# cvigilv/SimSpread.jl

Measured on AMD Instinct MI355X. Metric: predicted edges/sec + achieved HBM GB/s, W*R SpMM, higher is better.
Workload: dtype f32

## Files before the change

simspread.jl_amd/csrc/assemble.hip:

```cpp
#include <cstdlib>
#include <cstring>
#include <hip/hip_runtime.h>
#include <rocprim/rocprim.hpp>

#include "graph.hpp"

namespace ss {

static inline int grid_for(int64_t work, int block, int cap = 256 * 16) {
  int64_t g = ceil_div(work, block);
  if (g < 1) g = 1;
  if (g > cap) g = cap;
  return (int)g;
}

__global__ void scan_tail_kernel(const int* in, int* out, int64_t n) { out[n] = out[n - 1] + in[n - 1]; }

static int exclusive_scan_int(const int* in, int* out, int64_t n) {
  hipStream_t st = ctx().stream;
  if (n == 0) {
    SS_HIP(hipMemsetAsync(out, 0, sizeof(int), st));
    return SS_OK;
  }
  size_t bytes = 0;
// ... 289 lines not shown
  for (int64_t i = (int64_t)blockIdx.x * blockDim.x + threadIdx.x; i < n; i += (int64_t)gridDim.x * blockDim.x)
    atomicAdd(&hist[keys[i]], 1);
}

template <class T>
__global__ void gather_transpose_kernel(const int* __restrict__ perm, const int* __restrict__ rowid,
                                        const T* __restrict__ val, int64_t n, int* __restrict__ oidx,
                                        T* __restrict__ oval) {
  for (int64_t i = (int64_t)blockIdx.x * blockDim.x + threadIdx.x; i < n; i += (int64_t)gridDim.x * blockDim.x) {
    const int p = perm[i];
    oidx[i] = rowid[p];
    oval[i] = val[p];
  }
}

template <class T>
int csr_transpose(const DevCsr<T>& in, DevCsr<T>& out) {
  hipStream_t st = ctx().stream;
  out.rows = in.cols;
  out.cols = in.rows;
  out.nnz = in.nnz;
  out.binary = in.binary;
  SS_TRY(out.ptr.alloc(out.rows + 1));
  SS_TRY(out.idx.alloc(in.nnz));
  SS_TRY(out.val.alloc(in.nnz));
  const int64_t n = in.nnz;
  DevBuf<int> hist;
  SS_TRY(hist.alloc(out.rows + 1));
  SS_HIP(hipMemsetAsync(hist.p, 0, (out.rows + 1) * sizeof(int), st));
  if (n == 0) {
    SS_HIP(hipMemsetAsync(out.ptr.p, 0, (out.rows + 1) * sizeof(int), st));
    return SS_OK;
  }
  DevBuf<int> rowid, iota, keys_out, perm;
  SS_TRY(rowid.alloc(n));
  SS_TRY(iota.alloc(n));
  SS_TRY(keys_out.alloc(n));
  SS_TRY(perm.alloc(n));
  hipLaunchKernelGGL(expand_rows_kernel, dim3(grid_for(in.rows * 64, 256)), dim3(256), 0, st, in.ptr.p, in.rows,
                     rowid.p, iota.p);
  SS_LAUNCH_CHECK();
  int bits = 1;
  while ((1LL << bits) < in.cols && bits < 32) ++bits;
  size_t bytes = 0;
  SS_HIP(rocprim::radix_sort_pairs(nullptr, bytes, in.idx.p, keys_out.p, iota.p, perm.p, (size_t)n, 0u,
                                   (unsigned)bits, st));
  DevBuf<unsigned char> tmp;
  SS_TRY(tmp.alloc(bytes));
  SS_HIP(rocprim::radix_sort_pairs(tmp.p, bytes, in.idx.p, keys_out.p, iota.p, perm.p, (size_t)n, 0u,
                                   (unsigned)bits, st));
  hipLaunchKernelGGL(histogram_kernel, dim3(grid_for(n, 256)), dim3(256), 0, st, in.idx.p, n, hist.p);
  SS_LAUNCH_CHECK();
  SS_TRY(exclusive_scan_int(hist.p, out.ptr.p, out.rows));
  hipLaunchKernelGGL(gather_transpose_kernel<T>, dim3(grid_for(n, 256)), dim3(256), 0, st, perm.p, rowid.p,
                     in.val.p, n, out.idx.p, out.val.p);
  SS_LAUNCH_CHECK();
  SS_HIP(hipStreamSynchronize(st));
  return SS_OK;
}

__global__ void sell_width_kernel(const int* __restrict__ ptr, const int* __restrict__ idx, int64_t rows, int KC,
                                  int nslices, int nchunks, const int* __restrict__ vs, const int* __restrict__ ve,
                                  int* __restrict__ widthq) {
  const int lane = threadIdx.x & 63;
  const int64_t wave = ((int64_t)blockIdx.x * blockDim.x + threadIdx.x) >> 6;
  if (wave >= (int64_t)nslices * nchunks) return;
  const int c = (int)(wave / nslices), s = (int)(wave % nslices);
  const int64_t pos = (int64_t)s * 64 + lane;
  int n = 0;
  if (pos < rows) {
    int lo = vs ? vs[pos] : ptr[pos], hi = ve ? ve[pos] : ptr[pos + 1];
    const int64_t k0 = (int64_t)c * KC, k1 = k0 + KC;
    int a = lo, b = hi;
    while (a < b) { const int m = (a + b) >> 1; if (idx[m] < k0) a = m + 1; else b = m; }
    const int first = a;
    b = hi;
    while (a < b) { const int m = (a + b) >> 1; if (idx[m] < k1) a = m + 1; else b = m; }
    n = a - first;
  }
  for (int o = 32; o > 0; o >>= 1) { const int t = __shfl_xor(n, o); n = t > n ? t : n; }
  if (lane == 0) widthq[wave] = (n + 3) >> 2;
}

template <class T>
__global__ void sell_fill_kernel(const int* __restrict__ ptr, const int* __restrict__ idx, const T* __restrict__ val,
                                 int64_t rows, int KC, int nslices, int nchunks, const int* __restrict__ off,
                                 const int* __restrict__ vs, const int* __restrict__ ve,
                                 unsigned short* __restrict__ sidx, T* __restrict__ sval) {
  const int lane = threadIdx.x & 63;
  const int64_t wave = ((int64_t)blockIdx.x * blockDim.x + threadIdx.x) >> 6;
  if (wave >= (int64_t)nslices * nchunks) return;
  const int c = (int)(wave / nslices), s = (int)(wave % nslices);
  const int64_t pos = (int64_t)s * 64 + lane;
  int first = 0, n = 0;
  const int64_t k0 = (int64_t)c * KC, k1 = k0 + KC;
  if (pos < rows) {
    int lo = vs ? vs[pos] : ptr[pos], hi = ve ? ve[pos] : ptr[pos + 1];
    int a = lo, b = hi;
    while (a < b) { const int m = (a + b) >> 1; if (idx[m] < k0) a = m + 1; else b = m; }
    first = a;
    b = hi;
    while (a < b) { const int m = (a + b) >> 1; if (idx[m] < k1) a = m + 1; else b = m; }
    n = a - first;
  }
  const int o = off[wave], oe = off[wave + 1];
  for (int u = o; u < oe; ++u) {
    const int64_t base = ((int64_t)u * 64 + lane) * 4;
#pragma unroll
    for (int e = 0; e < 4; ++e) {
      const int p = (u - o) * 4 + e;
      const bool in = p < n;
      sidx[base + e] = in ? (unsigned short)(idx[first + p] - k0) : (unsigned short)KC;
      if (sval) sval[base + e] = in ? val[first + p] : T(0);
    }
  }
}

__device__ __forceinline__ void b128_group_of_lane(int lane, int& grp, int& gi) {
  const int l = lane & 31;
  int g, i;
  if (l < 4) { g = 0; i = l; }
  else if (l < 12) { g = 1; i = l - 4; }
  else if (l < 16) { g = 0; i = l - 8; }
  else if (l < 20) { g = 1; i = l - 8; }
  else if (l < 28) { g = 0; i = l - 12; }
  else { g = 1; i = l - 16; }
  grp = g + ((lane >> 5) << 1);
  gi = i;
}
__device__ __forceinline__ int b128_lane_of_group(int grp, int gi) {
  const int g = grp & 1;
  int l;
  if (g == 0) l = gi < 4 ? gi : (gi < 8 ? gi + 8 : gi + 12);
  else l = gi < 8 ? gi + 4 : (gi < 12 ? gi + 8 : gi + 16);
  return l + ((grp >> 1) << 5);
}

template <class T>
__global__ void __launch_bounds__(64) sell_fill_sched_kernel(const int* __restrict__ ptr, const int* __restrict__ idx,
                                                             const T* __restrict__ val, int64_t rows, int KC,
                                                             int nslices, int nchunks, const int* __restrict__ off,
                                                             const int* __restrict__ vs, const int* __restrict__ ve,
                                                             int* __restrict__ perm, unsigned short* __restrict__ sidx,
                                                             T* __restrict__ sval, int ncls, int npid) {
  __shared__ unsigned short cnt[64][17];
  __shared__ int cur[64][17];
  const int lane = threadIdx.x;
  const int64_t wave = blockIdx.x;
  const int c = (int)(wave / nslices), s = (int)(wave % nslices);
  const int64_t pos = (int64_t)s * 64 + lane;
  int first = 0, n = 0;
  const int64_t k0 = (int64_t)c * KC, k1 = k0 + KC;
  if (pos < rows) {
    int lo = vs ? vs[pos] : ptr[pos], hi = ve ? ve[pos] : ptr[pos + 1];
    int a = lo, b = hi;
    while (a < b) { const int m = (a + b) >> 1; if (idx[m] < k0) a = m + 1; else b = m; }
    first = a;
    b = hi;
    while (a < b) { const int m = (a + b) >> 1; if (idx[m] < k1) a = m + 1; else b = m; }
    n = a - first;
  }
  for (int q = 0; q < ncls; ++q) cnt[lane][q] = 0;
  for (int x = 0; x < n; ++x) cnt[lane][(idx[first + x] - k0) & (ncls - 1)]++;
  int run = first;
  for (int q = 0; q < ncls; ++q) { cur[lane][q] = run; run += cnt[lane][q]; }
  for (int x = 0; x < n; ++x) {
    const int q = (int)((idx[first + x] - k0) & (ncls - 1));
    perm[cur[lane][q]++] = first + x;
  }
  for (int q = 0; q < ncls; ++q) cur[lane][q] -= cnt[lane][q];

  int grp, gi;
  b128_group_of_lane(lane, grp, gi);
  const int o = off[wave], oe = off[wave + 1];
  int left = n;
  unsigned have = 0;
  for (int q = 0; q < ncls; ++q) have |= (cnt[lane][q] > 0 ? 1u : 0u) << q;
  const int psh = (lane & (npid - 1)) * ncls;
  for (int p = 0; p < (oe - o) * 4; ++p) {
    unsigned claimed = 0;
    int mine = -1;
    bool done = left == 0;
    for (int it = 0; it < 16; ++it) {
      if (__ballot(!done) == 0ull) break;
      const int rest = left > 4095 ? 4095 : left;
      int key = done ? 0x7fffffff : ((__popc(have & ~(claimed >> psh)) << 20) | ((4095 - rest) << 4) | gi);
#pragma unroll
      for (int m2 = 1; m2 < 16; m2 <<= 1) {
        const int other = __shfl(key, b128_lane_of_group(grp, gi ^ m2));
        key = other < key ? other : key;
      }
      const bool any = key != 0x7fffffff;
      const int wgi = key & 15;
      int choice = -1;
      if (any && !done && gi == wgi) {
        int best = -1, bestc = 0;
        for (int q = 0; q < ncls; ++q) {
          const int cq = cnt[lane][q];
          if (cq > bestc && !((claimed >> (psh + q)) & 1u)) { best = q; bestc = cq; }
        }
        if (best < 0)
          for (int q = 0; q < ncls; ++q) {
            const int cq = cnt[lane][q];
            if (cq > bestc) { best = q; bestc = cq; }
          }
        choice = best;
        mine = best;
        done = true;
      }
      const int wl = b128_lane_of_group(grp, wgi);
      const int ch = __shfl(choice, wl);
      if (any && ch >= 0) claimed |= 1u << ((wl & (npid - 1)) * ncls + ch);
    }
    const int64_t base = ((int64_t)(o + (p >> 2)) * 64 + lane) * 4 + (p & 3);
    if (mine >= 0) {
      const int e = perm[cur[lane][mine]];
      cur[lane][mine]++;
      cnt[lane][mine]--;
      if (cnt[lane][mine] == 0) have &= ~(1u << mine);
      --left;
      sidx[base] = (unsigned short)(idx[e] - k0);
      if (sval) sval[base] = val[e];
    } else {
      int q = 0;
      while (q < ncls - 1 && ((claimed >> (psh + q)) & 1u)) ++q;
      sidx[base] = (unsigned short)(KC + ((q - KC) & (ncls - 1)));
      if (sval) sval[base] = T(0);
    }
  }
}

__global__ void vrow_parts_kernel(const int* __restrict__ ptr, int64_t rows, int lmax, int* __restrict__ nparts) {
  for (int64_t i = (int64_t)blockIdx.x * blockDim.x + threadIdx.x; i < rows; i += (int64_t)gridDim.x * blockDim.x) {
    const int len = ptr[i + 1] - ptr[i];
    nparts[i] = len > lmax ? (len + lmax - 1) / lmax : 1;
  }
}
__global__ void vrow_fill_kernel(const int* __restrict__ ptr, const int* __restrict__ vfirst, int64_t rows, int lmax,
                                 int* __restrict__ vstart, int* __restrict__ vlen, int* __restrict__ iota) {
  for (int64_t r = (int64_t)blockIdx.x * blockDim.x + threadIdx.x; r < rows; r += (int64_t)gridDim.x * blockDim.x) {
    const int lo = ptr[r], hi = ptr[r + 1];
    for (int v = vfirst[r], p = 0; v < vfirst[r + 1]; ++v, ++p) {
      const int b = lo + p * lmax;
      const int e = (b + lmax < hi) ? b + lmax : hi;
      vstart[v] = b;
      vlen[v] = e > b ? e - b : 0;
      iota[v] = v;
    }
  }
}
__global__ void vrow_place_kernel(const int* __restrict__ perm, const int* __restrict__ vstart,
                                  const int* __restrict__ vlen, int64_t n, int* __restrict__ vs, int* __restrict__ ve,
                                  int* __restrict__ inv) {
  for (int64_t i = (int64_t)blockIdx.x * blockDim.x + threadIdx.x; i < n; i += (int64_t)gridDim.x * blockDim.x) {
    const int v = perm[i];
    vs[i] = vstart[v];
    ve[i] = vstart[v] + vlen[v];
    inv[v] = (int)i;
  }
}

template <class T>
int sell_build(const DevCsr<T>& in, int KCmax, DevSell<T>& out, int qt) {
  hipStream_t st = ctx().stream;
  if (qt <= 0) qt = sell_tile_width<T>();
  const int rowb = qt * (int)sizeof(T);
  if (rowb != 16 && rowb != 32) return fail(SS_EINVAL, "SELL tile rows must be 16 or 32 bytes");
  out.qt = qt;
  const int ncls = 256 / rowb, npid = rowb / 16;
  if (KCmax < 1 || KCmax > 65520) return fail(SS_EINVAL, "SELL chunk size out of range");
  out.rows = in.rows;
  out.cols = in.cols;
  out.binary = in.binary;
  out.KC = (int)((in.cols <= KCmax) ? (in.cols > 0 ? in.cols : 1) : KCmax);
  out.nchunks = (int)(in.cols > 0 ? ceil_div(in.cols, out.KC) : 1);
  out.nslices = (int)ceil_div(in.rows, 64);
  const int64_t nws = (int64_t)out.nslices * out.nchunks;
  SS_TRY(out.off.alloc(nws + 1));
  if (nws == 0) {
    SS_HIP(hipMemsetAsync(out.off.p, 0, sizeof(int), st));
    out.nquads = 0;
    SS_TRY(out.idx.alloc(0));
    SS_TRY(out.val.alloc(0));
    return SS_OK;
  }
  DevBuf<int> widthq;
  SS_TRY(widthq.alloc(nws));
  out.sorted = false;
  hipLaunchKernelGGL(sell_width_kernel, dim3((unsigned)ceil_div(nws * 64, 256)), dim3(256), 0, st, in.ptr.p, in.idx.p,
                     in.rows, out.KC, out.nslices, out.nchunks, (const int*)nullptr, (const int*)nullptr, widthq.p);
  SS_LAUNCH_CHECK();
  SS_TRY(exclusive_scan_int(widthq.p, out.off.p, nws));
  int nq = 0;
  SS_TRY(read_int(out.off.p + nws, &nq));
  out.vrows = in.rows;
  const bool skewed = ((double)nq - 0.4 * (double)nws) * 256.0 > 1.3 * (double)in.nnz + 65536.0;
  const bool want_sort = env_set("SS_SELL_SORT") ? env_int("SS_SELL_SORT", 0) != 0 : skewed;
  if (want_sort && in.rows > 64) {
    int64_t lmax = env_int("SS_SELL_LMAX", in.nnz / 4096);
    if (lmax < 256) lmax = 256;
    if (lmax > 65536) lmax = 65536;
    lmax &= ~3LL;
    DevBuf<int> nparts, vstart, vlen, vlen_sorted, iota, perm;
    SS_TRY(nparts.alloc(in.rows));
    SS_TRY(out.vfirst.alloc(in.rows + 1));
    hipLaunchKernelGGL(vrow_parts_kernel, dim3(grid_for(in.rows, 256)), dim3(256), 0, st, in.ptr.p, in.rows, (int)lmax,
                       nparts.p);
    SS_LAUNCH_CHECK();
    SS_TRY(exclusive_scan_int(nparts.p, out.vfirst.p, in.rows));
    int nv = 0;
    SS_TRY(read_int(out.vfirst.p + in.rows, &nv));
    out.vrows = nv;
    SS_TRY(vstart.alloc(nv));
    SS_TRY(vlen.alloc(nv));
    SS_TRY(vlen_sorted.alloc(nv));
    SS_TRY(iota.alloc(nv));
    SS_TRY(perm.alloc(nv));
    SS_TRY(out.vs.alloc(nv));
    SS_TRY(out.ve.alloc(nv));
    SS_TRY(out.inv.alloc(nv));
    hipLaunchKernelGGL(vrow_fill_kernel, dim3(grid_for(in.rows, 256)), dim3(256), 0, st, in.ptr.p, out.vfirst.p, in.rows,
                       (int)lmax, vstart.p, vlen.p, iota.p);
    SS_LAUNCH_CHECK();
    size_t bytes = 0;
    SS_HIP(rocprim::radix_sort_pairs_desc(nullptr, bytes, vlen.p, vlen_sorted.p, iota.p, perm.p, (size_t)nv, 0u, 32u, st));
    DevBuf<unsigned char> tmp;
    SS_TRY(tmp.alloc(bytes));
    SS_HIP(rocprim::radix_sort_pairs_desc(tmp.p, bytes, vlen.p, vlen_sorted.p, iota.p, perm.p, (size_t)nv, 0u, 32u, st));
    hipLaunchKernelGGL(vrow_place_kernel, dim3(grid_for(nv, 256)), dim3(256), 0, st, perm.p, vstart.p, vlen.p,
                       (int64_t)nv, out.vs.p, out.ve.p, out.inv.p);
    SS_LAUNCH_CHECK();
    out.sorted = true;
    out.nslices = (int)ceil_div((int64_t)nv, 64);
    const int64_t nws2 = (int64_t)out.nslices * out.nchunks;
    SS_TRY(out.off.alloc(nws2 + 1));
    SS_TRY(widthq.alloc(nws2));
    hipLaunchKernelGGL(sell_width_kernel, dim3((unsigned)ceil_div(nws2 * 64, 256)), dim3(256), 0, st, in.ptr.p,
                       in.idx.p, (int64_t)nv, out.KC, out.nslices, out.nchunks, (const int*)out.vs.p,
                       (const int*)out.ve.p, widthq.p);
    SS_LAUNCH_CHECK();
    SS_TRY(exclusive_scan_int(widthq.p, out.off.p, nws2));
    SS_TRY(read_int(out.off.p + nws2, &nq));
    SS_HIP(hipStreamSynchronize(st));
  }
  const int64_t nws_f = (int64_t)out.nslices * out.nchunks;
  if (nq < 0 || (int64_t)nq * 256 >= (1LL << 40)) return fail(SS_EUNSUPPORTED, "SELL storage too large");
  out.nquads = nq;
  const size_t slack = 8 * 256;
  SS_TRY(out.idx.alloc((size_t)nq * 256 + slack));
  SS_HIP(hipMemsetAsync(out.idx.p + (size_t)nq * 256, 0, slack * sizeof(unsigned short), st));
  if (!out.binary) {
    SS_TRY(out.val.alloc((size_t)nq * 256 + slack));
    SS_HIP(hipMemsetAsync(out.val.p + (size_t)nq * 256, 0, slack * sizeof(T), st));
  } else {
    out.val.release();
  }
  if (env_set("SS_SELL_PLAIN")) {
    hipLaunchKernelGGL(sell_fill_kernel<T>, dim3((unsigned)ceil_div(nws_f * 64, 256)), dim3(256), 0, st, in.ptr.p,
                       in.idx.p, in.val.p, out.vrows, out.KC, out.nslices, out.nchunks, out.off.p,
                       out.sorted ? (const int*)out.vs.p : (const int*)nullptr,
                       out.sorted ? (const int*)out.ve.p : (const int*)nullptr, out.idx.p,
                       out.binary ? (T*)nullptr : out.val.p);
    SS_LAUNCH_CHECK();
  } else {
    DevBuf<int> perm;
    SS_TRY(perm.alloc(in.nnz));
    hipLaunchKernelGGL(sell_fill_sched_kernel<T>, dim3((unsigned)nws_f), dim3(64), 0, st, in.ptr.p, in.idx.p, in.val.p,
                       out.vrows, out.KC, out.nslices, out.nchunks, out.off.p,
                       out.sorted ? (const int*)out.vs.p : (const int*)nullptr,
                       out.sorted ? (const int*)out.ve.p : (const int*)nullptr, perm.p, out.idx.p,
                       out.binary ? (T*)nullptr : out.val.p, ncls, npid);
    SS_LAUNCH_CHECK();
    SS_HIP(hipStreamSynchronize(st));
  }
  SS_HIP(hipStreamSynchronize(st));
  return SS_OK;
}

__device__ __forceinline__ void csell_subrow(const int* __restrict__ ptr, const int* __restrict__ idx, int64_t row,
                                             int64_t rows, int64_t k0, int KC, int& first, int& n) {
  first = 0; n = 0;
  if (row < rows) {
    const int lo = ptr[row], hi = ptr[row + 1];
    const int64_t k1 = k0 + KC;
    int a = lo, b = hi;
    while (a < b) { const int m = (a + b) >> 1; if (idx[m] < k0) a = m + 1; else b = m; }
    first = a;
    b = hi;
    while (a < b) { const int m = (a + b) >> 1; if (idx[m] < k1) a = m + 1; else b = m; }
    n = a - first;
  }
}

__global__ void __launch_bounds__(64) csell_count_kernel(const int* __restrict__ ptr, const int* __restrict__ idx,
                                                         int64_t rows, int KC, int nslices, int64_t nblocks,
                                                         unsigned short* __restrict__ np, int* __restrict__ steps,
                                                         int* __restrict__ pairs) {
  const int lane = threadIdx.x;
  for (int64_t b = blockIdx.x; b < nblocks; b += gridDim.x) {
    const int c = (int)(b / nslices), s = (int)(b % nslices);
    int first, n;
    csell_subrow(ptr, idx, (int64_t)s * 64 + lane, rows, (int64_t)c * KC, KC, first, n);
    const int p = (n + 1) >> 1;
    np[b * 64 + lane] = (unsigned short)p;
    int mx = p, sm = p;
#pragma unroll
    for (int o = 32; o > 0; o >>= 1) {
      const int m2 = __shfl_xor(mx, o);
      mx = m2 > mx ? m2 : mx;
      sm += __shfl_xor(sm, o);
    }
    if (lane == 0) { steps[b] = mx; pairs[b] = sm; }
  }
}

__global__ void csell_desc_kernel(const int* __restrict__ base, const int* __restrict__ steps, int64_t nblocks,
                                  int* __restrict__ desc) {
  for (int64_t b = (int64_t)blockIdx.x * blockDim.x + threadIdx.x; b <= nblocks; b += (int64_t)gridDim.x * blockDim.x) {
    desc[2 * b] = base[b];
    desc[2 * b + 1] = b < nblocks ? steps[b] : 0;
  }
}

template <class T, int ROWB>
__global__ void __launch_bounds__(64) csell_fill_kernel(const int* __restrict__ ptr, const int* __restrict__ idx,
                                                        const T* __restrict__ val, int64_t rows, int KC, int nslices,
                                                        int64_t nblocks, const int* __restrict__ desc, int* __restrict__ perm,
                                                        unsigned short* __restrict__ pidx16, T* __restrict__ pval) {
  constexpr int NPC = ROWB / 16, NCL = 256 / ROWB;
  __shared__ unsigned short cnt[64][NCL + 1];
  __shared__ int cur[64][NCL + 1];
  const int lane = threadIdx.x;
  int grp, gi;
  b128_group_of_lane(lane, grp, gi);
  for (int64_t b = blockIdx.x; b < nblocks; b += gridDim.x) {
    const int c = (int)(b / nslices), s = (int)(b % nslices);
    const int64_t k0 = (int64_t)c * KC;
    int first, n;
    csell_subrow(ptr, idx, (int64_t)s * 64 + lane, rows, k0, KC, first, n);
    const int64_t base = desc[2 * b];
    const int steps = desc[2 * b + 1];
    const int npl = (n + 1) >> 1;
    if (NCL > 1) {
      for (int q = 0; q < NCL; ++q) cnt[lane][q] = 0;
      for (int x = 0; x < n; ++x) cnt[lane][(idx[first + x] - k0) & (NCL - 1)]++;
      int run = first;
      for (int q = 0; q < NCL; ++q) { cur[lane][q] = run; run += cnt[lane][q]; }
      for (int x = 0; x < n; ++x) {
        const int q = (int)((idx[first + x] - k0) & (NCL - 1));
        perm[cur[lane][q]++] = first + x;
      }
      for (int q = 0; q < NCL; ++q) cur[lane][q] -= cnt[lane][q];
    }
    int left = n;
// ... 421 lines not shown
```

simspread.jl_amd/csrc/graph.hpp:

```cpp
#pragma once
#include "common.hpp"

#include <type_traits>

namespace ss {

template <class T>
struct DevCsr {
  int64_t rows = 0, cols = 0, nnz = 0;
  DevBuf<int> ptr;
  DevBuf<int> idx;
  DevBuf<T> val;
  bool binary = false;
};

template <class T>
struct DevSell {
  int64_t rows = 0, cols = 0;
  int KC = 0;
  int qt = 0;
  int nchunks = 0;
  int nslices = 0;
  int64_t nquads = 0;
  bool binary = false;
  DevBuf<int> off;
  DevBuf<unsigned short> idx;
  DevBuf<T> val;
  bool sorted = false;
  int64_t vrows = 0;
  DevBuf<int> vs, ve;
  DevBuf<int> vfirst;
  DevBuf<int> inv;
};

template <class T>
struct DevChunked {
  int64_t rows = 0, cols = 0, nnz = 0;
  int64_t stored = 0;
  bool binary = false;
  int SC = 0, nchunks = 0;
  int align = 1;
  DevBuf<int> off;
  DevBuf<unsigned short> idx;
  DevBuf<T> val;
  DevBuf<unsigned short> len;
  bool len_ok = false;
  float vmax = 0.f, vmin = 0.f;
};

template <class T>
struct DevCsell {
  int64_t rows = 0, cols = 0, nnz = 0;
  int KC = 0, nchunks = 0, nslices = 0;
  int QT = 0;
  bool binary = false;
  bool ok = false;
  int64_t npairs = 0;
  DevBuf<int> desc;
  DevBuf<unsigned short> np;
  DevBuf<unsigned> pidx;
  DevBuf<T> pval;
};

template <class T>
struct DenseSim {
  bool on = false;
  int64_t nq = 0, ns = 0, nf = 0;
  T alpha = T(0);
  bool weighted = true;
  DevBuf<T> Sq, Ss;
  DevBuf<T> inv_kf_m1;
  DevBuf<unsigned short> Bpl, Apl;
  int Bpl_np = 0;
  int64_t Bpl_Np = 0, Bpl_Kp = 0;
};

template <class T>
struct Graph {
  int64_t nq = 0, ns = 0, nf = 0, nt = 0;
  bool general = false;
  DenseSim<T> dense;
  DevCsr<T> Xq;
  DevCsr<T> Xs;
  DevCsr<T> XsT;
  DevCsr<T> Ys;
  DevCsr<T> YsT;
  DevBuf<int> kf, ks, kt;
  DevBuf<T> inv_kf, inv_ks, inv_kt;
  DevSell<T> W;
  int W_qt = 0;
  DevChunked<T> XsTc, YsTc;
  DevChunked<T> XsTb;
  DevBuf<T> Cq;
  DevBuf<T> Tws;
  DevBuf<T> Sws;
};

template <class T>
struct SpMat {
  DevCsr<T> csr;
  DevSell<T> sell;
  int sell_qt = 0;
  DevChunked<T> narrow[3];
  DevChunked<T> col[3];
  DevCsell<T> csell[6];
  bool csell_tried[6] = {false, false, false, false, false, false};
  DevBuf<T> partial;
};

template <class T>
// ... 283 lines not shown
```

simspread.jl_amd/csrc/kernels.hip:

```cpp
#include "graph.hpp"

namespace ss {

template <class T>
__global__ void cutoff_kernel(const T* __restrict__ X, int64_t rows, int64_t cols, int64_t ld, T alpha,
                              int weighted, T* __restrict__ out, int64_t ldo) {
  const int64_t total = rows * cols;
  for (int64_t i = (int64_t)blockIdx.x * blockDim.x + threadIdx.x; i < total;
       i += (int64_t)gridDim.x * blockDim.x) {
    const int64_t c = i / rows, r = i - c * rows;
    const T x = X[r + c * ld];
    out[r + c * ldo] = (x >= alpha) ? (weighted ? x : T(1)) : T(0);
  }
}

template <class T>
int launch_cutoff(const T* X, int64_t rows, int64_t cols, int64_t ld, T alpha, bool weighted, T* out, int64_t ldo) {
  if (rows * cols == 0) return SS_OK;
  hipLaunchKernelGGL(cutoff_kernel<T>, dim3(grid_1d(rows * cols, 256)), dim3(256), 0, ctx().stream, X, rows,
                     cols, ld, alpha, weighted ? 1 : 0, out, ldo);
  SS_LAUNCH_CHECK();
  return SS_OK;
}

template <class T>
__global__ void row_degree_kernel(const T* __restrict__ G, int64_t rows, int64_t cols, int64_t ld,
                                  int* __restrict__ deg) {
  for (int64_t r = (int64_t)blockIdx.x * blockDim.x + threadIdx.x; r < rows;
       r += (int64_t)gridDim.x * blockDim.x) {
    int n = 0;
    for (int64_t c = 0; c < cols; ++c) n += (G[r + c * ld] != T(0)) ? 1 : 0;
    deg[r] = n;
  }
}

template <class T>
int launch_row_degree(const T* G, int64_t rows, int64_t cols, int64_t ld, int* deg) {
  if (rows == 0) return SS_OK;
  hipLaunchKernelGGL(row_degree_kernel<T>, dim3(grid_1d(rows, 64)), dim3(64), 0, ctx().stream, G, rows, cols,
                     ld, deg);
  SS_LAUNCH_CHECK();
  return SS_OK;
}

template <class T>
__global__ void spread_dense_kernel(const T* __restrict__ G, int64_t rows, int64_t cols, int64_t ld,
                                    const int* __restrict__ deg, T* __restrict__ W, int64_t ldw) {
  const int64_t total = rows * cols;
  for (int64_t i = (int64_t)blockIdx.x * blockDim.x + threadIdx.x; i < total;
       i += (int64_t)gridDim.x * blockDim.x) {
    const int64_t c = i / rows, r = i - c * rows;
    const int d = deg[r];
    W[r + c * ldw] = d > 0 ? G[r + c * ld] / T(d) : T(0);
  }
}

template <class T>
int launch_spread_dense(const T* G, int64_t rows, int64_t cols, int64_t ld, const int* deg, T* W, int64_t ldw) {
  if (rows * cols == 0) return SS_OK;
  hipLaunchKernelGGL(spread_dense_kernel<T>, dim3(grid_1d(rows * cols, 256)), dim3(256), 0, ctx().stream, G,
                     rows, cols, ld, deg, W, ldw);
  SS_LAUNCH_CHECK();
  return SS_OK;
}

template <class T, int QT>
struct alignas(sizeof(T) * QT) Vec {
  T v[QT];
};

template <class T>
struct SellArgs {
  const int* off;
  const unsigned short* idx;
  const T* val;
  int nslices, nchunks, KC;
  int64_t K, M, B;
  const T* R;
  int64_t ldr;
  T* F;
  int64_t ldf;
  const int* clean_deg;
  const int* out_rows;
};

constexpr int SELL_THREADS = 1024;
constexpr int SELL_NB = 4;
constexpr int SELL_QT_F32_DEFAULT = 4;
constexpr int SELL_ZERO_ROWS = 16;
constexpr int SELL_STAGE_IT = 5;

template <int H>
__device__ __forceinline__ unsigned half_shl(unsigned x, unsigned sh) {
  unsigned r;
  if (H == 0)
    asm("v_lshlrev_b32_sdwa %0, %1, %2 dst_sel:DWORD dst_unused:UNUSED_PAD src0_sel:DWORD src1_sel:WORD_0"
        : "=v"(r) : "v"(sh), "v"(x));
  else
    asm("v_lshlrev_b32_sdwa %0, %1, %2 dst_sel:DWORD dst_unused:UNUSED_PAD src0_sel:DWORD src1_sel:WORD_1"
        : "=v"(r) : "v"(sh), "v"(x));
  return r;
}

template <class T, int QT, bool BIN>
__global__ void __launch_bounds__(SELL_THREADS) spmm_sell_kernel(SellArgs<T> a) {
  constexpr int RB = (int)sizeof(T) * QT, NP = RB / 16;
  constexpr int STAGE_IT = NP == 2 ? 2 : SELL_STAGE_IT;
  constexpr int NBQ = NP == 2 ? 2 : SELL_NB;
  constexpr unsigned TSH = NP == 2 ? 5 : 4;
  static_assert(RB == 16 || (RB == 32 && sizeof(T) == 4), "tile row must be 16 bytes, or 32 bytes of fp32");
  extern __shared__ __align__(16) unsigned char smem_raw[];
  using V = Vec<T, QT>;
  V* tile = reinterpret_cast<V*>(smem_raw);
  const int tid = threadIdx.x, lane = tid & 63, wave = tid >> 6, nwaves = blockDim.x >> 6;
  const int64_t b0 = (int64_t)blockIdx.x * QT;
  const unsigned pid = NP == 2 ? (unsigned)(lane & 1) : 0u;

  for (int c = 0; c < a.nchunks; ++c) {
    const int64_t k0 = (int64_t)c * a.KC;
    const int kn = (int)((a.K - k0 < a.KC) ? (a.K - k0) : a.KC);
    if (c) __syncthreads();
    for (int kb = 0; kb < a.KC + SELL_ZERO_ROWS; kb += STAGE_IT * SELL_THREADS) {
      T stg[STAGE_IT][QT];
      const int klast = kn > 0 ? kn - 1 : 0;
#pragma unroll
      for (int it = 0; it < STAGE_IT; ++it) {
        const int k = kb + tid + it * SELL_THREADS;
        const int kk = k < kn ? k : klast;
#pragma unroll
        for (int q = 0; q < QT; ++q) {
          const int64_t b = (b0 + q < a.B) ? b0 + q : a.B - 1;
          stg[it][q] = kn > 0 ? a.R[b * a.ldr + k0 + kk] : T(0);
        }
      }
#pragma unroll
      for (int it = 0; it < STAGE_IT; ++it) {
        const int k = kb + tid + it * SELL_THREADS;
        if (k < a.KC + SELL_ZERO_ROWS) {
          V v;
#pragma unroll
          for (int q = 0; q < QT; ++q) v.v[q] = (k < kn && b0 + q < a.B) ? stg[it][q] : T(0);
          tile[k] = v;
        }
      }
    }
    __syncthreads();

    const int* off = a.off + (int64_t)c * a.nslices;
    const bool last = (c == a.nchunks - 1);
    for (int s = wave + nwaves * (int)blockIdx.y; s < a.nslices; s += nwaves * (int)gridDim.y) {
      const int o = __builtin_amdgcn_readfirstlane(off[s]);
      const int oe = __builtin_amdgcn_readfirstlane(off[s + 1]);
      T acc[QT];
#pragma unroll
      for (int q = 0; q < QT; ++q) acc[q] = T(0);
      const int64_t m = (int64_t)s * 64 + lane;
      T fprev[QT];
#pragma unroll
      for (int q = 0; q < QT; ++q) {
        fprev[q] = T(0);
        if (NP == 1 && c && m < a.M && b0 + q < a.B)
          fprev[q] = a.F[(a.out_rows ? (int64_t)a.out_rows[b0 + q] : b0 + q) * a.ldf + m];
      }
      const ushort4* ip = reinterpret_cast<const ushort4*>(a.idx) + (int64_t)o * 64 + lane;
      const Vec<T, 4>* vp = reinterpret_cast<const Vec<T, 4>*>(a.val) + (int64_t)o * 64 + lane;
      const uint2* ipw = reinterpret_cast<const uint2*>(ip);
      const int nq = oe - o;
      uint2 ia[NBQ], ib[NBQ];
      Vec<T, 4> wa[NBQ], wb[NBQ];
      auto fetch = [&](uint2 (&iq)[NBQ], Vec<T, 4> (&wq)[NBQ], int base) __attribute__((always_inline)) {
#pragma unroll
        for (int j = 0; j < NBQ; ++j) {
          iq[j] = ipw[(int64_t)(base + j) * 64];
          if (!BIN) wq[j] = vp[(int64_t)(base + j) * 64];
        }
      };
      auto gather = [&](const uint2 (&iq)[NBQ], const Vec<T, 4> (&wq)[NBQ], int cnt) __attribute__((always_inline)) {
        constexpr int PV = 16 / (int)sizeof(T);
        typedef T NV __attribute__((ext_vector_type(PV)));
        using LV = const __attribute__((address_space(3))) NV*;
        const unsigned lb = pid << 4;
        auto row = [&](unsigned addr) __attribute__((always_inline)) {
          V r;
          if (NP == 1) {
            const NV n = *(LV)(uintptr_t)addr;
#pragma unroll
            for (int q = 0; q < PV; ++q) r.v[q] = n[q];
          } else {
            const unsigned a0 = addr | lb;
            const NV n0 = *(LV)(uintptr_t)a0;
            const NV n1 = *(LV)(uintptr_t)(a0 ^ 16u);
#pragma unroll
            for (int q = 0; q < PV; ++q) { r.v[q] = n0[q]; r.v[PV + q] = n1[q]; }
          }
          return r;
        };
#pragma unroll
        for (int j = 0; j < NBQ; ++j) {
          if (j >= cnt) break;
          const V t0 = row(half_shl<0>(iq[j].x, TSH));
          const V t1 = row(half_shl<1>(iq[j].x, TSH));
          const V t2 = row(half_shl<0>(iq[j].y, TSH));
          const V t3 = row(half_shl<1>(iq[j].y, TSH));
          if (BIN) {
#pragma unroll
            for (int q = 0; q < QT; ++q) acc[q] += (t0.v[q] + t1.v[q]) + (t2.v[q] + t3.v[q]);
          } else {
#pragma unroll
            for (int q = 0; q < QT; ++q) {
              acc[q] = fma(wq[j].v[0], t0.v[q], acc[q]);
              acc[q] = fma(wq[j].v[1], t1.v[q], acc[q]);
              acc[q] = fma(wq[j].v[2], t2.v[q], acc[q]);
              acc[q] = fma(wq[j].v[3], t3.v[q], acc[q]);
            }
          }
          if (NP == 2) __builtin_amdgcn_sched_barrier(0);
        }
      };
      fetch(ia, wa, 0);
      fetch(ib, wb, NBQ);
      int u = 0;
      for (; u + 2 * NBQ <= nq; u += 2 * NBQ) {
        gather(ia, wa, NBQ);
        fetch(ia, wa, u + 2 * NBQ);
        gather(ib, wb, NBQ);
        fetch(ib, wb, u + 3 * NBQ);
      }
      {
        const int rest = nq - u;
        if (rest > 0) gather(ia, wa, rest < NBQ ? rest : NBQ);
        if (rest > NBQ) gather(ib, wb, rest - NBQ);
      }
      if (m < a.M) {
        const bool flag = last && a.clean_deg != nullptr && a.clean_deg[m] == 0;
#pragma unroll
        for (int q = 0; q < QT; ++q) {
          if (b0 + q < a.B) {
            T* f = a.F + (a.out_rows ? (int64_t)a.out_rows[b0 + q] : b0 + q) * a.ldf + m;
            const T mine = NP == 2 ? (pid ? acc[q ^ (QT / 2)] : acc[q]) : acc[q];
            const T r = mine + ((NP == 2 && c) ? *f : fprev[q]);
            *f = flag ? T(-99) : r;
          }
        }
      }
    }
  }
}

template <> int sell_tile_width<float>() {
  const int v = (int)env_int("SS_SELL_QT", 0);
  if (v == 4 || v == 8) return v;
  return SELL_QT_F32_DEFAULT;
}
template <> int sell_tile_width<double>() { return 2; }

template <class T>
int sell_max_chunk(int qt) {
  int64_t kc = (int64_t)(160 * 1024) / ((int64_t)qt * (int64_t)sizeof(T)) - SELL_ZERO_ROWS;
  if (kc > 65535 - (SELL_ZERO_ROWS - 1)) kc = 65535 - (SELL_ZERO_ROWS - 1);
  return (int)kc;
}

template <class T>
int launch_spmm_sell(const DevSell<T>& W, const T* R, int64_t ldr, int64_t B, T* F, int64_t ldf,
                     const int* clean_deg, const int* out_rows) {
  if (B <= 0 || W.rows <= 0) return SS_OK;
  path_add(W.sorted ? "spmm_sell_sorted" : "spmm_sell");
  const int QT = W.qt > 0 ? W.qt : (sizeof(T) == 4 ? 4 : 2);
  SellArgs<T> a{};
  a.off = W.off.p;
  a.idx = W.idx.p;
  a.val = W.val.p;
  a.nslices = W.nslices;
  a.nchunks = W.nchunks;
  a.KC = W.KC;
  a.K = W.cols;
  a.M = W.sorted ? W.vrows : W.rows;
  a.B = B;
  a.R = R;
  a.ldr = ldr;
  a.F = F;
  a.ldf = ldf;
  a.clean_deg = clean_deg;
  a.out_rows = out_rows;
  const size_t lds = (size_t)(W.KC + SELL_ZERO_ROWS) * QT * sizeof(T);
  if (lds > (size_t)160 * 1024) return fail(SS_EINVAL, "SELL chunk does not fit the LDS tile of %d columns", QT);
  const unsigned gx = (unsigned)ceil_div(B, QT);
  unsigned gy = 1;
  if ((int)gx < 2 * ctx().num_cu) {
    gy = (unsigned)ceil_div(2 * ctx().num_cu, (int64_t)gx);
    const unsigned maxy = (unsigned)ceil_div(W.nslices, SELL_THREADS / 64);
    if (gy > maxy) gy = maxy > 0 ? maxy : 1;
  }
  const dim3 grid(gx, gy);
  auto prepare = [](const void* fn) -> int {
    hipFuncAttributes fa{};
    SS_HIP(hipFuncGetAttributes(&fa, fn));
    if (fa.sharedSizeBytes != 0)
      return fail(SS_EUNSUPPORTED, "spmm_sell_kernel was built with %zu bytes of static LDS: its tile-relative LDS "
                  "addresses need the dynamic segment at LDS address 0", (size_t)fa.sharedSizeBytes);
    SS_HIP(hipFuncSetAttribute(fn, hipFuncAttributeMaxDynamicSharedMemorySize, 160 * 1024));
    return SS_OK;
  };
#define SS_SELL_LAUNCH(QTV, BINV, SLOT)                                                                      \
  do {                                                                                                       \
    static std::atomic<bool> attr_done{false};                                                               \
    if (!attr_done) {                                                                                        \
      SS_TRY(prepare(reinterpret_cast<const void*>(&spmm_sell_kernel<T, QTV, BINV>)));                       \
      attr_done = true;                                                                                      \
    }                                                                                                        \
    hipLaunchKernelGGL((spmm_sell_kernel<T, QTV, BINV>), grid, dim3(SELL_THREADS), lds, ctx().stream, a);    \
  } while (0)
  if constexpr (sizeof(T) == 4) {
    if (QT == 8) { if (W.binary) SS_SELL_LAUNCH(8, true, 0); else SS_SELL_LAUNCH(8, false, 1); }
    else if (QT == 4) { if (W.binary) SS_SELL_LAUNCH(4, true, 2); else SS_SELL_LAUNCH(4, false, 3); }
    else return fail(SS_EINVAL, "SELL tile width must be 4 or 8 (fp32)");
  } else {
    if (QT != 2) return fail(SS_EINVAL, "SELL tile width must be 2 (fp64)");
    if (W.binary) SS_SELL_LAUNCH(2, true, 0); else SS_SELL_LAUNCH(2, false, 1);
  }
#undef SS_SELL_LAUNCH
  SS_LAUNCH_CHECK();
  return SS_OK;
}

template <class T>
struct NarrowArgs {
  const int* off;
  const unsigned short* idx;
  const T* val;
  int64_t M, K;
  int KC, nchunks, B;
  const T* R;
  int64_t ldr;
  T* F;
  int64_t ldf;
  T* P;
};

constexpr int NARROW_THREADS = 1024;

template <int CTRL, int ROW_MASK = 0xF>
__device__ __forceinline__ float dpp_add(float v) {
  return v + __int_as_float(__builtin_amdgcn_update_dpp(0, __float_as_int(v), CTRL, ROW_MASK, 0xF, false));
}
template <int CTRL, int ROW_MASK = 0xF>
__device__ __forceinline__ double dpp_add(double v) {
  const long long b = __double_as_longlong(v);
  const int lo = __builtin_amdgcn_update_dpp(0, (int)(b & 0xffffffffll), CTRL, ROW_MASK, 0xF, false);
  const int hi = __builtin_amdgcn_update_dpp(0, (int)(b >> 32), CTRL, ROW_MASK, 0xF, false);
  return v + __longlong_as_double(((long long)hi << 32) | (unsigned int)lo);
}
template <int GL, class T>
__device__ __forceinline__ T lane_group_sum(T v) {
  static_assert(GL == 8 || GL == 16 || GL == 32 || GL == 64, "group of 8, 16, 32 or 64 lanes");
  v = dpp_add<0xB1>(v);
  v = dpp_add<0x4E>(v);
  v = dpp_add<0x141>(v);
  if constexpr (GL >= 16) v = dpp_add<0x140>(v);
  if constexpr (GL >= 32) v = dpp_add<0x142, 0xA>(v);
  if constexpr (GL >= 64) v = dpp_add<0x143, 0xC>(v);
  return v;
}

template <class T, int VEC, int GL, int UR, int NBQ>
__global__ void __launch_bounds__(NARROW_THREADS) spmm_chunked_narrow_kernel(NarrowArgs<T> a) {
  constexpr int BV = VEC;
// ... 688 lines not shown
```

Measured before the change: 48.79 billion.

## Lend long SELL rows' excess nonzeros to short rows within a slice

Adds a planning kernel that, per SELL slice and column chunk, picks a shorter padded width Q2 and a split point Q1. Rows longer than 4*Q2 hand their excess nonzeros to rows that finish by Q1. Those receiver lanes compute partial sums for the donor rows in the tail quads, and the SpMM kernel adds them back with ds_bpermute before writing out. The aim is to cut padding in slices with skewed row lengths, so less index and value data is stored and read. The cost is extra metadata reads, cross-lane reduction work in the SpMM kernel, and a more complex build step.

```diff
diff --git a/simspread.jl_amd/csrc/assemble.hip b/simspread.jl_amd/csrc/assemble.hip
--- a/simspread.jl_amd/csrc/assemble.hip
+++ b/simspread.jl_amd/csrc/assemble.hip
@@ -395,6 +395,71 @@
   if (lane == 0) widthq[wave] = (n + 3) >> 2;
 }
 
+__global__ void sell_plan_kernel(const int* __restrict__ ptr, const int* __restrict__ idx, int64_t rows, int KC,
+                                 int nslices, int nchunks, int* __restrict__ widthq, int* __restrict__ q1,
+                                 int* __restrict__ nlend) {
+  const int lane = threadIdx.x & 63;
+  const int64_t wave = ((int64_t)blockIdx.x * blockDim.x + threadIdx.x) >> 6;
+  if (wave >= (int64_t)nslices * nchunks) return;
+  const int c = (int)(wave / nslices), s = (int)(wave % nslices);
+  const int64_t pos = (int64_t)s * 64 + lane;
+  int n = 0;
+  if (pos < rows) {
+    const int lo = ptr[pos], hi = ptr[pos + 1];
+    const int64_t k0 = (int64_t)c * KC, k1 = k0 + KC;
+    int a = lo, b = hi;
+    while (a < b) { const int m = (a + b) >> 1; if (idx[m] < k0) a = m + 1; else b = m; }
+    const int first = a;
+    b = hi;
+    while (a < b) { const int m = (a + b) >> 1; if (idx[m] < k1) a = m + 1; else b = m; }
+    n = a - first;
+  }
+  int nmax = n, tot = n;
+  for (int o = 32; o > 0; o >>= 1) {
+    const int t = __shfl_xor(nmax, o);
+    nmax = t > nmax ? t : nmax;
+    tot += __shfl_xor(tot, o);
+  }
+  const int qmax = (nmax + 3) >> 2;
+  auto valid = [&](int Q1, int Q2, int nrecv) {
+    const int cap = 4 * (Q2 - Q1);
+    const int e = n > 4 * Q2 ? n - 4 * Q2 : 0;
+    const int need = (e + cap - 1) / cap;
+    if (__ballot(need > SELL_LEND_R) != 0ull) return false;
+    const int sum = __popcll(__ballot(need >= 1)) + __popcll(__ballot(need >= 2)) + __popcll(__ballot(need >= 3));
+    return sum <= nrecv;
+  };
+  static_assert(SELL_LEND_R == 3, "the sum of the needs above counts up to three receivers per donor");
+  int bq1 = qmax, bq2 = qmax;
+  const int qmin = (tot + 255) >> 8;
+  for (int Q1 = 0; Q1 < qmax - 1; Q1 += SELL_Q1_STEP) {
+    const int nrecv = __popcll(__ballot(n <= 4 * Q1));
+    if (nrecv == 0) continue;
+    int lo = Q1 + 1 > qmin ? Q1 + 1 : qmin;
+    int hi = bq2 < qmax - 1 ? bq2 : qmax - 1;
+    if (lo > hi || !valid(Q1, hi, nrecv)) continue;
+    while (lo < hi) {
+      const int mid = (lo + hi) >> 1;
+      if (valid(Q1, mid, nrecv)) hi = mid; else lo = mid + 1;
+    }
+    bq1 = Q1;
+    bq2 = hi;
+  }
+  if (lane == 0) {
+    widthq[wave] = bq2;
+    q1[wave] = bq1;
+    if (bq1 < bq2) atomicAdd(nlend, 1);
+  }
+}
+
+__global__ void sell_meta_plain_kernel(const int* __restrict__ off, int64_t nws, int* __restrict__ q1,
+                                       unsigned* __restrict__ rec) {
+  for (int64_t i = (int64_t)blockIdx.x * blockDim.x + threadIdx.x; i < nws * 64; i += (int64_t)gridDim.x * blockDim.x) {
+    rec[i] = SELL_REC_NONE;
+    if ((i & 63) == 0) q1[i >> 6] = off[(i >> 6) + 1] - off[i >> 6];
+  }
+}
+
 template <class T>
 __global__ void sell_fill_kernel(const int* __restrict__ ptr, const int* __restrict__ idx, const T* __restrict__ val,
                                  int64_t rows, int KC, int nslices, int nchunks, const int* __restrict__ off,
@@ -455,9 +520,12 @@
                                                              int nslices, int nchunks, const int* __restrict__ off,
                                                              const int* __restrict__ vs, const int* __restrict__ ve,
                                                              int* __restrict__ perm, unsigned short* __restrict__ sidx,
-                                                             T* __restrict__ sval, int ncls, int npid) {
+                                                             T* __restrict__ sval, int ncls, int npid,
+                                                             const int* __restrict__ q1, unsigned* __restrict__ rec) {
   __shared__ unsigned short cnt[64][17];
   __shared__ int cur[64][17];
+  __shared__ int sh_exc[64], sh_start[64];
+  __shared__ unsigned char sh_recv[64][4];
   const int lane = threadIdx.x;
   const int64_t wave = blockIdx.x;
   const int c = (int)(wave / nslices), s = (int)(wave % nslices);
@@ -490,10 +558,8 @@
   unsigned have = 0;
   for (int q = 0; q < ncls; ++q) have |= (cnt[lane][q] > 0 ? 1u : 0u) << q;
   const int psh = (lane & (npid - 1)) * ncls;
-  for (int p = 0; p < (oe - o) * 4; ++p) {
-    unsigned claimed = 0;
+  auto pick = [&](unsigned& claimed, bool done, bool may_wait) {
     int mine = -1;
-    bool done = left == 0;
     for (int it = 0; it < 16; ++it) {
       if (__ballot(!done) == 0ull) break;
       const int rest = left > 4095 ? 4095 : left;
@@ -512,7 +578,7 @@
           const int cq = cnt[lane][q];
           if (cq > bestc && !((claimed >> (psh + q)) & 1u)) { best = q; bestc = cq; }
         }
-        if (best < 0)
+        if (best < 0 && !may_wait)
           for (int q = 0; q < ncls; ++q) {
             const int cq = cnt[lane][q];
             if (cq > bestc) { best = q; bestc = cq; }
@@ -525,21 +591,89 @@
       const int ch = __shfl(choice, wl);
       if (any && ch >= 0) claimed |= 1u << ((wl & (npid - 1)) * ncls + ch);
     }
+    return mine;
+  };
+  auto place = [&](int64_t base, int mine, int step) {
+    const int e = perm[cur[lane][mine]];
+    cur[lane][mine] += step;
+    cnt[lane][mine]--;
+    if (cnt[lane][mine] == 0) have &= ~(1u << mine);
+    --left;
+    sidx[base] = (unsigned short)(idx[e] - k0);
+    if (sval) sval[base] = val[e];
+  };
+  auto pad = [&](int64_t base, unsigned claimed) {
+    int q = 0;
+    while (q < ncls - 1 && ((claimed >> (psh + q)) & 1u)) ++q;
+    sidx[base] = (unsigned short)(KC + ((q - KC) & (ncls - 1)));
+    if (sval) sval[base] = T(0);
+  };
+  for (int p = 0; p < (oe - o) * 4; ++p) {
+    unsigned claimed = 0;
+    const int mine = pick(claimed, left == 0, false);
     const int64_t base = ((int64_t)(o + (p >> 2)) * 64 + lane) * 4 + (p & 3);
-    if (mine >= 0) {
-      const int e = perm[cur[lane][mine]];
-      cur[lane][mine]++;
-      cnt[lane][mine]--;
-      if (cnt[lane][mine] == 0) have &= ~(1u << mine);
-      --left;
-      sidx[base] = (unsigned short)(idx[e] - k0);
-      if (sval) sval[base] = val[e];
-    } else {
-      int q = 0;
-      while (q < ncls - 1 && ((claimed >> (psh + q)) & 1u)) ++q;
-      sidx[base] = (unsigned short)(KC + ((q - KC) & (ncls - 1)));
-      if (sval) sval[base] = T(0);
-    }
+    if (mine >= 0) place(base, mine, 1);
+    else pad(base, claimed);
+  }
+  const int Q2 = oe - o, Q1 = q1 ? q1[wave] : Q2;
+  if (!rec) return;
+  if (Q1 >= Q2) {
+    rec[wave * 64 + lane] = SELL_REC_NONE;
+    return;
+  }
+  const int cap = 4 * (Q2 - Q1);
+  const int exc = left;
+  sh_exc[lane] = exc;
+  sh_recv[lane][0] = sh_recv[lane][1] = sh_recv[lane][2] = 0xff;
+  __syncthreads();
+  int start = -1;
+  if (exc > 0) {
+    start = 0;
+    for (int l = 0; l < 64; ++l) {
+      const int ol = sh_exc[l];
+      if (ol > exc || (ol == exc && l < lane)) start += (ol + cap - 1) / cap;
+    }
+  }
+  sh_start[lane] = start;
+  __syncthreads();
+  const bool can_recv = n <= 4 * Q1;
+  const int ridx = __popcll(__ballot(can_recv) & ((1ull << lane) - 1ull));
+  int donor = -1, part = 0, parts = 1;
+  if (can_recv)
+    for (int l = 0; l < 64; ++l) {
+      const int need = (sh_exc[l] + cap - 1) / cap;
+      if (need > 0 && ridx >= sh_start[l] && ridx < sh_start[l] + need) { donor = l; part = ridx - sh_start[l]; parts = need; }
+    }
+  if (donor >= 0 && part < SELL_LEND_R) sh_recv[donor][part] = (unsigned char)lane;
+  __syncthreads();
+  rec[wave * 64 + lane] = (unsigned)sh_recv[lane][0] | ((unsigned)sh_recv[lane][1] << 8) | ((unsigned)sh_recv[lane][2] << 16) |
+                          (donor >= 0 ? 1u << 24 : 0u);
+  left = 0;
+  have = 0;
+  if (donor >= 0) {
+    int pre = 0;
+    for (int q = 0; q < ncls; ++q) {
+      const int cd = cnt[donor][q];
+      const int f = pre + (((part - pre) % parts) + parts) % parts;
+      const int cq = f < pre + cd ? (pre + cd - 1 - f) / parts + 1 : 0;
+      cnt[lane][q] = (unsigned short)cq;
+      cur[lane][q] = cur[donor][q] + (f - pre);
+      if (cq > 0) have |= 1u << q;
+      left += cq;
+      pre += cd;
+    }
+  }
+  __syncthreads();
+  for (int p = Q1 * 4; p < Q2 * 4; ++p) {
+    const int64_t base = ((int64_t)(o + (p >> 2)) * 64 + lane) * 4 + (p & 3);
+    const unsigned short held = sidx[base];
+    const bool fixed = held < KC;
+    unsigned claimed = fixed ? 1u << (psh + (held & (ncls - 1))) : 0u;
+#pragma unroll
+    for (int m2 = 1; m2 < 16; m2 <<= 1) claimed |= (unsigned)__shfl((int)claimed, b128_lane_of_group(grp, gi ^ m2));
+    const int mine = pick(claimed, !(donor >= 0 && left > 0), left < Q2 * 4 - p);
+    if (mine >= 0) place(base, mine, parts);
+    else if (!fixed) pad(base, claimed);
   }
 }
 
@@ -657,6 +791,37 @@
     SS_HIP(hipStreamSynchronize(st));
   }
   const int64_t nws_f = (int64_t)out.nslices * out.nchunks;
+  out.lends = false;
+  const bool plain = env_set("SS_SELL_PLAIN");
+  if (rowb == 16) {
+    SS_TRY(out.q1.alloc(nws_f + 1));
+    SS_TRY(out.rec.alloc(nws_f * 64));
+    if (!out.sorted && !plain && env_int("SS_SELL_LEND", 1) != 0) {
+      SS_HIP(hipMemsetAsync(out.q1.p + nws_f, 0, sizeof(int), st));
+      hipLaunchKernelGGL(sell_plan_kernel, dim3((unsigned)ceil_div(nws_f * 64, 256)), dim3(256), 0, st, in.ptr.p, in.idx.p,
+                         in.rows, out.KC, out.nslices, out.nchunks, widthq.p, out.q1.p, out.q1.p + nws_f);
+      SS_LAUNCH_CHECK();
+      int nlend = 0;
+      SS_TRY(read_int(out.q1.p + nws_f, &nlend));
+      if (nlend > 0) {
+        out.lends = true;
+        SS_TRY(exclusive_scan_int(widthq.p, out.off.p, nws_f));
+        SS_TRY(read_int(out.off.p + nws_f, &nq));
+      }
+    }
+    if (!out.lends) {
+      hipLaunchKernelGGL(sell_meta_plain_kernel, dim3(grid_for(nws_f * 64, 256)), dim3(256), 0, st, (const int*)out.off.p,
+                         nws_f, out.q1.p, out.rec.p);
+      SS_LAUNCH_CHECK();
+    }
+  } else {
+    out.q1.release();
+    out.rec.release();
+  }
+  if (env_int("SS_SELL_STATS", 0) != 0)
+    fprintf(stderr, "sell_build: rows %lld cols %lld nnz %lld chunks %d slices %d quads %d slots_per_nnz %.4f lend %d sorted %d\n",
+            (long long)in.rows, (long long)in.cols, (long long)in.nnz, out.nchunks, out.nslices, nq,
+            in.nnz > 0 ? (double)nq * 256.0 / (double)in.nnz : 0.0, out.lends ? 1 : 0, out.sorted ? 1 : 0);
   if (nq < 0 || (int64_t)nq * 256 >= (1LL << 40)) return fail(SS_EUNSUPPORTED, "SELL storage too large");
   out.nquads = nq;
   const size_t slack = 8 * 256;
@@ -682,7 +847,7 @@
                        out.vrows, out.KC, out.nslices, out.nchunks, out.off.p,
                        out.sorted ? (const int*)out.vs.p : (const int*)nullptr,
                        out.sorted ? (const int*)out.ve.p : (const int*)nullptr, perm.p, out.idx.p,
-                       out.binary ? (T*)nullptr : out.val.p, ncls, npid);
+                       out.binary ? (T*)nullptr : out.val.p, ncls, npid, (const int*)out.q1.p, out.rec.p);
     SS_LAUNCH_CHECK();
     SS_HIP(hipStreamSynchronize(st));
   }
diff --git a/simspread.jl_amd/csrc/graph.hpp b/simspread.jl_amd/csrc/graph.hpp
--- a/simspread.jl_amd/csrc/graph.hpp
+++ b/simspread.jl_amd/csrc/graph.hpp
@@ -13,6 +13,10 @@
   DevBuf<T> val;
   bool binary = false;
 };
+
+constexpr int SELL_Q1_STEP = 8;
+constexpr int SELL_LEND_R = 3;
+constexpr unsigned SELL_REC_NONE = 0x00ffffffu;
 
 template <class T>
 struct DevSell {
@@ -26,6 +30,9 @@
   DevBuf<int> off;
   DevBuf<unsigned short> idx;
   DevBuf<T> val;
+  DevBuf<int> q1;
+  DevBuf<unsigned> rec;
+  bool lends = false;
   bool sorted = false;
   int64_t vrows = 0;
   DevBuf<int> vs, ve;
diff --git a/simspread.jl_amd/csrc/kernels.hip b/simspread.jl_amd/csrc/kernels.hip
--- a/simspread.jl_amd/csrc/kernels.hip
+++ b/simspread.jl_amd/csrc/kernels.hip
@@ -82,10 +82,13 @@
   int64_t ldf;
   const int* clean_deg;
   const int* out_rows;
+  const int* q1;
+  const unsigned* rec;
 };
 
 constexpr int SELL_THREADS = 1024;
 constexpr int SELL_NB = 4;
+static_assert(SELL_Q1_STEP == 2 * SELL_NB, "a lending slice's first part must end with a turn of the gather loop");
 constexpr int SELL_QT_F32_DEFAULT = 4;
 constexpr int SELL_ZERO_ROWS = 16;
 constexpr int SELL_STAGE_IT = 5;
@@ -162,6 +165,12 @@
         if (NP == 1 && c && m < a.M && b0 + q < a.B)
           fprev[q] = a.F[(a.out_rows ? (int64_t)a.out_rows[b0 + q] : b0 + q) * a.ldf + m];
       }
+      int q1 = oe - o;
+      unsigned rec = SELL_REC_NONE;
+      if (NP == 1) {
+        q1 = __builtin_amdgcn_readfirstlane(a.q1[(int64_t)c * a.nslices + s]);
+        rec = a.rec[((int64_t)c * a.nslices + s) * 64 + lane];
+      }
       const ushort4* ip = reinterpret_cast<const ushort4*>(a.idx) + (int64_t)o * 64 + lane;
       const Vec<T, 4>* vp = reinterpret_cast<const Vec<T, 4>*>(a.val) + (int64_t)o * 64 + lane;
       const uint2* ipw = reinterpret_cast<const uint2*>(ip);
@@ -219,17 +228,45 @@
       };
       fetch(ia, wa, 0);
       fetch(ib, wb, NBQ);
+      const bool recv = NP == 1 && ((rec >> 24) & 1u);
+      T own[QT];
+#pragma unroll
+      for (int q = 0; q < QT; ++q) own[q] = T(0);
       int u = 0;
       for (; u + 2 * NBQ <= nq; u += 2 * NBQ) {
         gather(ia, wa, NBQ);
         fetch(ia, wa, u + 2 * NBQ);
         gather(ib, wb, NBQ);
         fetch(ib, wb, u + 3 * NBQ);
+        if (NP == 1 && u + 2 * NBQ == q1) {
+#pragma unroll
+          for (int q = 0; q < QT; ++q) { own[q] = recv ? acc[q] : own[q]; acc[q] = recv ? T(0) : acc[q]; }
+        }
       }
       {
         const int rest = nq - u;
         if (rest > 0) gather(ia, wa, rest < NBQ ? rest : NBQ);
         if (rest > NBQ) gather(ib, wb, rest - NBQ);
+      }
+      if (NP == 1 && q1 < nq) {
+        constexpr int NW = (int)(sizeof(T) * QT / 4);
+        int lent[NW];
+        __builtin_memcpy(lent, acc, sizeof(lent));
+#pragma unroll
+        for (int r = 0; r < SELL_LEND_R; ++r) {
+          const unsigned src = (rec >> (8 * r)) & 0xffu;
+          if (__ballot(src != 0xffu) == 0ull) break;
+          const int from = (int)((src != 0xffu ? src : (unsigned)lane) << 2);
+          int got[NW];
+#pragma unroll
+          for (int w = 0; w < NW; ++w) got[w] = __builtin_amdgcn_ds_bpermute(from, lent[w]);
+          T add[QT];
+          __builtin_memcpy(add, got, sizeof(got));
+#pragma unroll
+          for (int q = 0; q < QT; ++q) acc[q] = src != 0xffu ? acc[q] + add[q] : acc[q];
+        }
+#pragma unroll
+        for (int q = 0; q < QT; ++q) acc[q] = recv ? own[q] : acc[q];
       }
       if (m < a.M) {
         const bool flag = last && a.clean_deg != nullptr && a.clean_deg[m] == 0;
@@ -283,6 +320,9 @@
   a.ldf = ldf;
   a.clean_deg = clean_deg;
   a.out_rows = out_rows;
+  a.q1 = W.q1.p;
+  a.rec = W.rec.p;
+  if (W.lends) path_add("sell_lend");
   const size_t lds = (size_t)(W.KC + SELL_ZERO_ROWS) * QT * sizeof(T);
   if (lds > (size_t)160 * 1024) return fail(SS_EINVAL, "SELL chunk does not fit the LDS tile of %d columns", QT);
   const unsigned gx = (unsigned)ceil_div(B, QT);
```

After: 49.57 billion, median of 6. 1.02x the previous value.
